# Aster32/GAN-DANet

Hardware: AMD Instinct MI355X
Metric: train samples/sec (G+D step) on 256x256 tiles (higher is better)
Workload: dtype bf16; 1 GPU; full G+D train step, 8ch 256x256 -> 1024x1024 tiles, batch 32/GPU (global 32), perceptual=on, SSIM evaluated, AdamW x2; survey_config=3, per_gpu_batch=32, global_batch=32, tile=256, parallelism=dp1

## Files before the change

### gan-danet_amd/csrc/conv3x3.hip

```cpp
#include "common.h"
#include "tile_mma.h"
#include "../../include/gandanet.h"

namespace {

using gd::acc_row;
using gd::bf16x8_native_t;
typedef unsigned int u32x4_t __attribute__((ext_vector_type(4)));

constexpr int TW = 32;
constexpr int PW = TW + 2;
constexpr int CK = 32;
constexpr int LD = CK + 8;

__global__ void pack_w_kernel(const float* __restrict__ a, long a_sm, long a_sc, long a_st, int M, int Ck, int flip,
                              int BM, int nchunks, unsigned short* __restrict__ wp, long total) {
    for (long i = (long)blockIdx.x * blockDim.x + threadIdx.x; i < total; i += (long)gridDim.x * blockDim.x) {
        const int cc = (int)(i % CK);
        long t = i / CK;
        const int mm = (int)(t % BM);
        t /= BM;
        const int tap = (int)(t % 9);
        t /= 9;
        const int chunk = (int)(t % nchunks);
        const int mt = (int)(t / nchunks);
        const int m = mt * BM + mm, c = chunk * CK + cc;
        float v = 0.f;
        if (m < M && c < Ck) v = a[(long)m * a_sm + (long)c * a_sc + (long)(flip ? 8 - tap : tap) * a_st];
        wp[i] = gd_f2bf(v);
    }
}

template <int BM, int TH, int S>
__global__ __launch_bounds__(256, 2) void conv3x3_halo_kernel(const gd_conv_desc d, const unsigned short* __restrict__ wp,
                                                             int tiles_x, int nchunks) {
    constexpr int WAVES_M = 2, WAVES_N = 2;
    constexpr int TM = BM / (32 * WAVES_M);
    constexpr int TN = TH / WAVES_N;
    constexpr int PH = S * (TH - 1) + 3;
    constexpr int PWk = S * (TW - 1) + 3;
    constexpr int NPIX = PH * PWk;
    constexpr int WCHUNKS = 3 * BM * CK / 8;
    constexpr int WPT = WCHUNKS / 256;
    static_assert(WCHUNKS % 256 == 0, "weight stage must divide evenly");

    __shared__ __attribute__((aligned(16))) unsigned short patch[NPIX * LD];
    __shared__ __attribute__((aligned(16))) unsigned short wts[3 * BM * LD];

    const int tid = threadIdx.x, lane = tid & 63, wave = tid >> 6;
    const int r = lane & 31, h = lane >> 5;
    const int wm = wave >> 1, wn = wave & 1;
    const int b = blockIdx.z;
    const int mt = blockIdx.y;
    const int ty = blockIdx.x / tiles_x, tx = blockIdx.x - ty * tiles_x;
    const int y0 = ty * TH, x0 = tx * TW;
    const int H = d.Hi, W = d.Wi;
    const int Ho = d.Ho, Wo = d.Wo;
    const long HW = (long)H * W, HWo = (long)Ho * Wo;
    const float* ximg = d.x + (long)b * d.x_bs;

    f32x16_t acc[TM][TN];
#pragma unroll
    for (int i = 0; i < TM; ++i)
#pragma unroll
        for (int j = 0; j < TN; ++j)
#pragma unroll
            for (int e = 0; e < 16; ++e) acc[i][j][e] = 0.f;

    const unsigned short* wbase = wp + (long)mt * nchunks * 9 * BM * CK;
    u32x4_t wreg[WPT];
    auto load_w = [&](int chunk, int ky) {
        const u32x4_t* src = reinterpret_cast<const u32x4_t*>(wbase + ((long)chunk * 9 + ky * 3) * BM * CK);
#pragma unroll
        for (int i = 0; i < WPT; ++i) wreg[i] = src[tid + i * 256];
    };
    auto store_w = [&]() {
#pragma unroll
        for (int i = 0; i < WPT; ++i) {
            const int v = tid + i * 256;
            const int row = v >> 2, q = v & 3;
            *reinterpret_cast<u32x4_t*>(wts + row * LD + q * 8) = wreg[i];
        }
    };

    for (int chunk = 0; chunk < nchunks; ++chunk) {
        const int c0 = chunk * CK;
        load_w(chunk, 0);
        for (int w = tid; w < 2 * NPIX; w += 256) {
            const int half = w >= NPIX ? 1 : 0;
            const int pix = w - half * NPIX;
            const int py = pix / PWk, px = pix - py * PWk;
            const int iy = S * y0 - 1 + py, ix = S * x0 - 1 + px;
            const bool inside = iy >= 0 && iy < H && ix >= 0 && ix < W;
            const int cb = c0 + half * 16;
            const float* p = ximg + (long)cb * HW + (long)iy * W + ix;
            unsigned int* dst = reinterpret_cast<unsigned int*>(patch + pix * LD + half * 16);
#pragma unroll
            for (int j = 0; j < 8; ++j) {
                const int c = cb + 2 * j;
                float v0 = 0.f, v1 = 0.f;
                if (inside) {
                    if (c < d.Ck) v0 = p[(long)(2 * j) * HW];
                    if (c + 1 < d.Ck) v1 = p[(long)(2 * j + 1) * HW];
                    if (d.in_scale) {
                        if (c < d.Ck) {
                            v0 = fmaf(v0, d.in_scale[c], d.in_shift[c]);
                            if (d.in_relu) v0 = fmaxf(v0, 0.f);
                        }
                        if (c + 1 < d.Ck) {
                            v1 = fmaf(v1, d.in_scale[c + 1], d.in_shift[c + 1]);
                            if (d.in_relu) v1 = fmaxf(v1, 0.f);
                        }
                    }
                }
                dst[j] = gd_pack_bf2(v0, v1);
            }
        }
        for (int ky = 0; ky < 3; ++ky) {
            store_w();
            __syncthreads();
            if (ky < 2) load_w(chunk, ky + 1);
#pragma unroll
            for (int kx = 0; kx < 3; ++kx) {
#pragma unroll
                for (int ks = 0; ks < CK / 16; ++ks) {
                    bf16x8_t fa[TM], fb[TN];
#pragma unroll
                    for (int i = 0; i < TM; ++i)
                        fa[i] = *reinterpret_cast<const bf16x8_t*>(wts + (kx * BM + wm * TM * 32 + i * 32 + r) * LD +
                                                                  ks * 16 + 8 * h);
#pragma unroll
                    for (int j = 0; j < TN; ++j)
                        fb[j] = *reinterpret_cast<const bf16x8_t*>(patch + (((wn * TN + j) * S + ky) * PWk + r * S + kx) * LD +
                                                                  ks * 16 + 8 * h);
#pragma unroll
                    for (int i = 0; i < TM; ++i)
#pragma unroll
                        for (int j = 0; j < TN; ++j)
                            acc[i][j] = __builtin_amdgcn_mfma_f32_32x32x16_bf16(
                                __builtin_bit_cast(bf16x8_native_t, fa[i]), __builtin_bit_cast(bf16x8_native_t, fb[j]),
                                acc[i][j], 0, 0, 0);
                }
            }
            __syncthreads();
        }
    }

    const float alpha = d.alpha ? *d.alpha : 1.f;
    const int ox = x0 + r;
    if (ox < Wo) {
#pragma unroll
        for (int j = 0; j < TN; ++j) {
            const int oy = y0 + wn * TN + j;
            if (oy >= Ho) continue;
            const long pn = (long)oy * Wo + ox;
#pragma unroll
            for (int i = 0; i < TM; ++i)
#pragma unroll
                for (int e = 0; e < 16; ++e) {
                    const int m = mt * BM + wm * TM * 32 + i * 32 + acc_row(e, h);
                    if (m >= d.M) continue;
                    float v = acc[i][j][e] * alpha;
                    if (d.bias) v += d.bias[m];
                    if (d.res) v += d.res[(long)b * d.res_bs + (long)m * HWo + pn];
                    if (d.act == GD_ACT_RELU) v = fmaxf(v, 0.f);
                    else if (d.act == GD_ACT_LEAKY02) v = v >= 0.f ? v : 0.2f * v;
                    float* yp = reinterpret_cast<float*>(d.y) + (long)b * d.y_bs + (long)m * HWo + pn;
                    if (d.accumulate) v += *yp;
                    *yp = v;
                }
        }
    }
}

}

static inline int pick_bm(int M, int Ck) {
    if (Ck <= CK && M > 64) return 128;
    return (M <= 64 || (M % 128 != 0 && M % 128 <= 64)) ? 64 : 128;
}

extern "C" size_t gd_conv3x3_ws_bytes(int M, int Ck) {
    const int bm = pick_bm(M, Ck);
    const long mtiles = (M + bm - 1) / bm, nchunks = (Ck + CK - 1) / CK;
    return (size_t)(mtiles * bm * nchunks * CK * 9 * 2);
}

extern "C" int gd_conv3x3_eligible(const gd_conv_desc* d) {
    if (!(d && d->ks == 3 && d->pad == 1 && d->out_layout == 0 && !d->out_bf16 && d->precision == GD_PREC_BF16 &&
          d->a_bs == 0 && (d->Mstore == 0 || d->Mstore == d->M) && d->sub_step <= 1))
        return 0;
    if (d->stride == 1) return d->Hi == d->Ho && d->Wi == d->Wo;
    return d->stride == 2 && !d->transposed && (d->Hi - 1) / 2 + 1 == d->Ho && (d->Wi - 1) / 2 + 1 == d->Wo;
}

extern "C" int gd_conv3x3(const gd_conv_desc* dp, void* ws, size_t ws_bytes, void* stream) {
    GD_CHECK_ARG(dp && ws, "gd_conv3x3: null argument");
    GD_CHECK_ARG(gd_conv3x3_eligible(dp), "gd_conv3x3: descriptor not eligible (needs 3x3, pad 1, stride 1 or forward stride 2, bf16, fp32 NCHW out)");
    const gd_conv_desc& d = *dp;
    GD_CHECK_ARG(d.B > 0 && d.B <= 65535 && d.M > 0 && d.Ck > 0 && d.Hi > 0 && d.Wi > 0, "gd_conv3x3: bad sizes");
    GD_CHECK_ARG(d.a && d.x && d.y, "gd_conv3x3: null tensor");
    GD_CHECK_ARG((d.in_scale == nullptr) == (d.in_shift == nullptr), "gd_conv3x3: in_scale/in_shift must come together");
    GD_CHECK_ARG(ws_bytes >= gd_conv3x3_ws_bytes(d.M, d.Ck), "gd_conv3x3: workspace too small");
    hipStream_t s = (hipStream_t)stream;
    const int bm = pick_bm(d.M, d.Ck);
    const int mtiles = (d.M + bm - 1) / bm, nchunks = (d.Ck + CK - 1) / CK;
    const long total = (long)mtiles * nchunks * 9 * bm * CK;
    {
        int blocks = (int)((total + 255) / 256);
        if (blocks > 2048) blocks = 2048;
        hipLaunchKernelGGL(pack_w_kernel, dim3(blocks), dim3(256), 0, s, d.a, d.a_sm, d.a_sc, d.a_st, d.M, d.Ck,
                           d.transposed ? 1 : 0, bm, nchunks, (unsigned short*)ws, total);
    }
    const int th = d.stride == 1 ? 8 : 4;
    const int tiles_x = (d.Wo + TW - 1) / TW, tiles_y = (d.Ho + th - 1) / th;
    GD_CHECK_ARG((long)tiles_x * tiles_y < (1L << 31), "gd_conv3x3: image too large");
    dim3 grid(tiles_x * tiles_y, mtiles, d.B);
    const unsigned short* wpk = (const unsigned short*)ws;
    if (d.stride == 1) {
        if (bm == 64) hipLaunchKernelGGL((conv3x3_halo_kernel<64, 8, 1>), grid, dim3(256), 0, s, d, wpk, tiles_x, nchunks);
        else hipLaunchKernelGGL((conv3x3_halo_kernel<128, 8, 1>), grid, dim3(256), 0, s, d, wpk, tiles_x, nchunks);
    } else {
        if (bm == 64) hipLaunchKernelGGL((conv3x3_halo_kernel<64, 4, 2>), grid, dim3(256), 0, s, d, wpk, tiles_x, nchunks);
        else hipLaunchKernelGGL((conv3x3_halo_kernel<128, 4, 2>), grid, dim3(256), 0, s, d, wpk, tiles_x, nchunks);
    }
    GD_LAUNCH_CHECK();
    return 0;
}

namespace {

struct NhwcConvArgs {
    const unsigned short* x;
    const unsigned short* wp;
    const float* bias;
    const unsigned short* mask;
    const unsigned short* res;
    unsigned short* y;
    float* y32;
    long y32_bs;
    int H, W, Ho, Wo, K, M, act, tiles_x, nchunks;
    float slope;
    int osplit;
    int epi_lds;
};

template <int BM, int S, int EPI = 0>
__global__ __launch_bounds__(256, 2) void conv3x3_nhwc_kernel(const NhwcConvArgs a) {
    constexpr int TH = S == 1 ? 8 : 4;
    constexpr int WAVES_M = 2, WAVES_N = 2;
    constexpr int TM = BM / (32 * WAVES_M);
    constexpr int TN = TH / WAVES_N;
    constexpr int PH = S * (TH - 1) + 3, PWk = S * (TW - 1) + 3, NPIX = PH * PWk;
    constexpr int WCHUNKS = 3 * BM * CK / 8;
    constexpr int WPT = WCHUNKS / 256;
    constexpr int NIT = (4 * NPIX + 255) / 256;
    static_assert(WCHUNKS % 256 == 0, "weight stage must divide evenly");

    __shared__ __attribute__((aligned(16))) unsigned short patch[NPIX * LD];
    __shared__ __attribute__((aligned(16))) unsigned short wts[3 * BM * LD];

    const int tid = threadIdx.x, lane = tid & 63, wave = tid >> 6;
    const int r = lane & 31, h = lane >> 5;
    const int wm = wave >> 1, wn = wave & 1;
    const int b = blockIdx.z, mt = blockIdx.y;
    const int ty = blockIdx.x / a.tiles_x, tx = blockIdx.x - ty * a.tiles_x;
    const int y0 = ty * TH, x0 = tx * TW;
    const int H = a.H, W = a.W, K = a.K;
    const unsigned short* ximg = a.x + (long)b * H * W * K;

    f32x16_t acc[TM][TN];
#pragma unroll
    for (int i = 0; i < TM; ++i)
#pragma unroll
        for (int j = 0; j < TN; ++j)
#pragma unroll
            for (int e = 0; e < 16; ++e) acc[i][j][e] = 0.f;

    const unsigned short* wbase = a.wp + (long)mt * a.nchunks * 9 * BM * CK;
    u32x4_t wreg[WPT];
    auto load_w = [&](int chunk, int ky) {
        const u32x4_t* src = reinterpret_cast<const u32x4_t*>(wbase + ((long)chunk * 9 + ky * 3) * BM * CK);
#pragma unroll
        for (int i = 0; i < WPT; ++i) wreg[i] = src[tid + i * 256];
    };
    auto store_w = [&]() {
#pragma unroll
        for (int i = 0; i < WPT; ++i) {
            const int v = tid + i * 256;
            const int row = v >> 2, q = v & 3;
            *reinterpret_cast<u32x4_t*>(wts + row * LD + q * 8) = wreg[i];
        }
    };

    unsigned int goff[NIT], inmask = 0, slotmask = 0;
    int loff[NIT];
#pragma unroll
    for (int it = 0; it < NIT; ++it) {
        const int w = tid + it * 256;
        const int pix = w >> 2, q = w & 3;
        const int py = pix / PWk, px = pix - py * PWk;
        const int iy = S * y0 - 1 + py, ix = S * x0 - 1 + px;
        const bool slot = w < 4 * NPIX;
        const bool inside = slot && iy >= 0 && iy < H && ix >= 0 && ix < W;
        loff[it] = pix * LD + q * 8;
        goff[it] = inside ? (unsigned int)(((long)iy * W + ix) * K + q * 8) : 0u;
        inmask |= inside ? (1u << it) : 0u;
        slotmask |= slot ? (1u << it) : 0u;
    }
    u32x4_t raw[NIT];
    auto load_patch = [&](int chunk) {
        const unsigned short* base = ximg + chunk * CK;
#pragma unroll
        for (int it = 0; it < NIT; ++it) {
            const int q = (tid + it * 256) & 3;
            const u32x4_t z = {0u, 0u, 0u, 0u};
            raw[it] = (((inmask >> it) & 1u) && chunk * CK + q * 8 < K) ? *reinterpret_cast<const u32x4_t*>(base + goff[it]) : z;
        }
    };
    auto store_patch = [&]() {
#pragma unroll
        for (int it = 0; it < NIT; ++it)
            if ((slotmask >> it) & 1u) *reinterpret_cast<u32x4_t*>(patch + loff[it]) = raw[it];
    };

    load_patch(0);
    store_patch();
    for (int chunk = 0; chunk < a.nchunks; ++chunk) {
        load_w(chunk, 0);
#pragma unroll
        for (int ky = 0; ky < 3; ++ky) {
            store_w();
            __syncthreads();
            if (ky == 0 && chunk + 1 < a.nchunks) load_patch(chunk + 1);
            if (ky < 2) load_w(chunk, ky + 1);
#pragma unroll
            for (int kx = 0; kx < 3; ++kx) {
#pragma unroll
                for (int ks = 0; ks < CK / 16; ++ks) {
                    bf16x8_t fa[TM], fb[TN];
#pragma unroll
                    for (int i = 0; i < TM; ++i)
                        fa[i] = *reinterpret_cast<const bf16x8_t*>(wts + (kx * BM + wm * TM * 32 + i * 32 + r) * LD +
                                                                  ks * 16 + 8 * h);
#pragma unroll
                    for (int j = 0; j < TN; ++j)
                        fb[j] = *reinterpret_cast<const bf16x8_t*>(patch + (((wn * TN + j) * S + ky) * PWk + r * S + kx) * LD +
                                                                  ks * 16 + 8 * h);
#pragma unroll
                    for (int i = 0; i < TM; ++i)
#pragma unroll
                        for (int j = 0; j < TN; ++j)
                            acc[i][j] = __builtin_amdgcn_mfma_f32_32x32x16_bf16(
                                __builtin_bit_cast(bf16x8_native_t, fa[i]), __builtin_bit_cast(bf16x8_native_t, fb[j]),
                                acc[i][j], 0, 0, 0);
                }
            }
            __syncthreads();
        }
        if (chunk + 1 < a.nchunks) store_patch();
    }

    if constexpr (EPI == 1) {
        constexpr int SLD = LD;
        static_assert(4 * 2 * 32 * SLD <= NPIX * LD, "per-wave scratch must fit in the patch image");
        unsigned short* scr = patch + wave * (2 * 32 * SLD);
        const int RS = a.osplit ? 3 * a.M : a.M;
        const int ox = x0 + r;
#pragma unroll
        for (int j = 0; j < TN; ++j) {
            const int oy = y0 + wn * TN + j;
            if (oy >= a.Ho) continue;
            const long prow = ((long)b * a.Ho + oy) * a.Wo;
#pragma unroll
            for (int i = 0; i < TM; ++i) {
                const int mbase = mt * BM + wm * TM * 32 + i * 32;
                if (mbase >= a.M) continue;
#pragma unroll
                for (int g = 0; g < 4; ++g) {
                    const int m = mbase + 8 * g + 4 * h;
                    const bool ok = ox < a.Wo && m < a.M;
                    float v[4];
#pragma unroll
                    for (int k = 0; k < 4; ++k) {
                        v[k] = acc[i][j][4 * g + k];
                        if (a.bias && ok) v[k] += a.bias[m + k];
                        if (a.act == 1) v[k] = fmaxf(v[k], 0.f);
                        else if (a.act == 2) v[k] = v[k] > 0.f ? v[k] : v[k] * a.slope;
                    }
                    if (ok) {
                        const long pbase = (prow + ox) * RS;
                        if (a.mask) {
                            const uint2 mk = *reinterpret_cast<const uint2*>(a.mask + pbase + m);
                            if (!((mk.x & 0x7FFFu) && !(mk.x & 0x8000u))) v[0] = 0.f;
                            if (!((mk.x >> 16) & 0x7FFFu) || (mk.x >> 31)) v[1] = 0.f;
                            if (!((mk.y & 0x7FFFu) && !(mk.y & 0x8000u))) v[2] = 0.f;
                            if (!((mk.y >> 16) & 0x7FFFu) || (mk.y >> 31)) v[3] = 0.f;
                        }
                        if (a.res) {
#pragma unroll
                            for (int part = 0; part < 2; ++part) {
                                if (part && !a.osplit) break;
                                const uint2 rr = *reinterpret_cast<const uint2*>(a.res + pbase + part * a.M + m);
                                v[0] += gd_bf2f((unsigned short)(rr.x & 0xFFFFu));
                                v[1] += gd_bf2f((unsigned short)(rr.x >> 16));
                                v[2] += gd_bf2f((unsigned short)(rr.y & 0xFFFFu));
                                v[3] += gd_bf2f((unsigned short)(rr.y >> 16));
                            }
                        }
                    }
                    uint2 hi, lo = make_uint2(0u, 0u);
                    if (a.osplit) {
                        gd_split_bf2(v[0], v[1], hi.x, lo.x);
                        gd_split_bf2(v[2], v[3], hi.y, lo.y);
                        *reinterpret_cast<uint2*>(scr + 32 * SLD + r * SLD + 8 * g + 4 * h) = lo;
                    } else {
                        hi.x = gd_pack_bf2(v[0], v[1]);
                        hi.y = gd_pack_bf2(v[2], v[3]);
                    }
                    *reinterpret_cast<uint2*>(scr + r * SLD + 8 * g + 4 * h) = hi;
                }
#pragma unroll
                for (int pass = 0; pass < 2; ++pass) {
                    const int px = pass * 16 + (lane >> 2), c8 = (lane & 3) * 8;
                    const int oxp = x0 + px, m = mbase + c8;
                    if (oxp < a.Wo && m < a.M) {
                        unsigned short* dst = a.y + (prow + oxp) * RS + m;
                        const u32x4_t vh = *reinterpret_cast<const u32x4_t*>(scr + px * SLD + c8);
                        *reinterpret_cast<u32x4_t*>(dst) = vh;
                        if (a.osplit) {
                            *reinterpret_cast<u32x4_t*>(dst + a.M) = *reinterpret_cast<const u32x4_t*>(scr + 32 * SLD + px * SLD + c8);
                            *reinterpret_cast<u32x4_t*>(dst + 2 * a.M) = vh;
                        }
                    }
                }
            }
        }
        return;
    }

    const int ox = x0 + r;
    if (ox < a.Wo) {
#pragma unroll
        for (int j = 0; j < TN; ++j) {
            const int oy = y0 + wn * TN + j;
            if (oy >= a.Ho) continue;
            const long pbase = (((long)b * a.Ho + oy) * a.Wo + ox) * (a.osplit ? 3 * a.M : a.M);
#pragma unroll
            for (int i = 0; i < TM; ++i)
#pragma unroll
                for (int g = 0; g < 4; ++g) {
                    const int m = mt * BM + wm * TM * 32 + i * 32 + 8 * g + 4 * h;
                    if (m >= a.M) continue;
                    float v[4];
#pragma unroll
                    for (int k = 0; k < 4; ++k) {
                        v[k] = acc[i][j][4 * g + k];
                        if (a.bias) v[k] += a.bias[m + k];
                        if (a.act == 1) v[k] = fmaxf(v[k], 0.f);
                        else if (a.act == 2) v[k] = v[k] > 0.f ? v[k] : v[k] * a.slope;
                    }
                    if (a.mask) {
                        const uint2 mk = *reinterpret_cast<const uint2*>(a.mask + pbase + m);
                        if (!((mk.x & 0x7FFFu) && !(mk.x & 0x8000u))) v[0] = 0.f;
                        if (!((mk.x >> 16) & 0x7FFFu) || (mk.x >> 31)) v[1] = 0.f;
                        if (!((mk.y & 0x7FFFu) && !(mk.y & 0x8000u))) v[2] = 0.f;
                        if (!((mk.y >> 16) & 0x7FFFu) || (mk.y >> 31)) v[3] = 0.f;
                    }
                    if (a.res) {
#pragma unroll
                        for (int part = 0; part < 2; ++part) {
                            if (part && !a.osplit) break;
                            const uint2 rr = *reinterpret_cast<const uint2*>(a.res + pbase + part * a.M + m);
                            v[0] += gd_bf2f((unsigned short)(rr.x & 0xFFFFu));
                            v[1] += gd_bf2f((unsigned short)(rr.x >> 16));
                            v[2] += gd_bf2f((unsigned short)(rr.y & 0xFFFFu));
                            v[3] += gd_bf2f((unsigned short)(rr.y >> 16));
                        }
                    }
                    if (a.y32) {
                        float* yp = a.y32 + (long)b * a.y32_bs + (long)m * a.Ho * a.Wo + (long)oy * a.Wo + ox;
#pragma unroll
                        for (int k = 0; k < 4; ++k) yp[(long)k * a.Ho * a.Wo] = v[k];
                        continue;
                    }
                    uint2 o;
                    if (a.osplit) {
                        uint2 lo;
                        gd_split_bf2(v[0], v[1], o.x, lo.x);
                        gd_split_bf2(v[2], v[3], o.y, lo.y);
                        *reinterpret_cast<uint2*>(a.y + pbase + a.M + m) = lo;
                        *reinterpret_cast<uint2*>(a.y + pbase + 2 * a.M + m) = o;
                    } else {
                        o.x = gd_pack_bf2(v[0], v[1]);
                        o.y = gd_pack_bf2(v[2], v[3]);
                    }
                    *reinterpret_cast<uint2*>(a.y + pbase + m) = o;
                }
        }
    }
}

struct NhwcDgrad2Args {
    const unsigned short* dy;
    const unsigned short* wp;
    const unsigned short* act;
    unsigned short* dx;
    int H, W, Ho, Wo, K, M, tiles_x, nchunks;
    float slope;
    int split;
};

__global__ __launch_bounds__(256, 2) void conv3x3_nhwc_dgrad2_kernel(const NhwcDgrad2Args a) {
    constexpr int BM = 64, TH = 4;
    constexpr int TN = TH / 2;
    constexpr int PH = TH + 1, PWd = TW + 1, NPIX = PH * PWd;
    constexpr int WPT = 3 * BM * CK / 8 / 256;
    constexpr int NIT = (4 * NPIX + 255) / 256;

    __shared__ __attribute__((aligned(16))) unsigned short patch[NPIX * LD];
    __shared__ __attribute__((aligned(16))) unsigned short wts[3 * BM * LD];

    const int tid = threadIdx.x, lane = tid & 63, wave = tid >> 6;
    const int r = lane & 31, h = lane >> 5;
    const int wm = wave >> 1, wn = wave & 1;
    const int b = blockIdx.z, mt = blockIdx.y;
    const int ty = blockIdx.x / a.tiles_x, tx = blockIdx.x - ty * a.tiles_x;
    const int u0 = ty * TH, v0 = tx * TW;
    const int Ho = a.Ho, Wo = a.Wo, M = a.M;
    const unsigned short* dyimg = a.dy + (long)b * Ho * Wo * M;

    f32x16_t acc[4][TN];
#pragma unroll
    for (int c = 0; c < 4; ++c)
#pragma unroll
        for (int j = 0; j < TN; ++j)
#pragma unroll
            for (int e = 0; e < 16; ++e) acc[c][j][e] = 0.f;

    const unsigned short* wbase = a.wp + (long)mt * a.nchunks * 9 * BM * CK;
    u32x4_t wreg[WPT];
    auto load_w = [&](int chunk, int ky) {
        const u32x4_t* src = reinterpret_cast<const u32x4_t*>(wbase + ((long)chunk * 9 + ky * 3) * BM * CK);
#pragma unroll
        for (int i = 0; i < WPT; ++i) wreg[i] = src[tid + i * 256];
    };
    auto store_w = [&]() {
#pragma unroll
        for (int i = 0; i < WPT; ++i) {
            const int v = tid + i * 256;
            *reinterpret_cast<u32x4_t*>(wts + (v >> 2) * LD + (v & 3) * 8) = wreg[i];
        }
    };

    unsigned int goff[NIT], inmask = 0, slotmask = 0;
    int loff[NIT];
#pragma unroll
    for (int it = 0; it < NIT; ++it) {
        const int w = tid + it * 256;
        const int pix = w >> 2, q = w & 3;
        const int py = pix / PWd, px = pix - py * PWd;
        const int iy = u0 + py, ix = v0 + px;
        const bool slot = w < 4 * NPIX;
        const bool inside = slot && iy < Ho && ix < Wo;
        loff[it] = pix * LD + q * 8;
        goff[it] = inside ? (unsigned int)(((long)iy * Wo + ix) * M + q * 8) : 0u;
        inmask |= inside ? (1u << it) : 0u;
        slotmask |= slot ? (1u << it) : 0u;
    }
    u32x4_t raw[NIT];
    auto load_patch = [&](int chunk) {
        const unsigned short* base = dyimg + chunk * CK;
#pragma unroll
        for (int it = 0; it < NIT; ++it) {
            const int q = (tid + it * 256) & 3;
            const u32x4_t z = {0u, 0u, 0u, 0u};
            raw[it] = (((inmask >> it) & 1u) && chunk * CK + q * 8 < M) ? *reinterpret_cast<const u32x4_t*>(base + goff[it]) : z;
        }
    };
    auto store_patch = [&]() {
#pragma unroll
        for (int it = 0; it < NIT; ++it)
            if ((slotmask >> it) & 1u) *reinterpret_cast<u32x4_t*>(patch + loff[it]) = raw[it];
    };

    load_patch(0);
    store_patch();
    for (int chunk = 0; chunk < a.nchunks; ++chunk) {
        load_w(chunk, 0);
#pragma unroll
        for (int ky = 0; ky < 3; ++ky) {
            store_w();
            __syncthreads();
            if (ky == 0 && chunk + 1 < a.nchunks) load_patch(chunk + 1);
            if (ky < 2) load_w(chunk, ky + 1);
            const int py = (ky + 1) & 1, oy = ky == 0 ? 1 : 0;
#pragma unroll
            for (int kx = 0; kx < 3; ++kx) {
                const int px = (kx + 1) & 1, ox = kx == 0 ? 1 : 0;
#pragma unroll
                for (int ks = 0; ks < CK / 16; ++ks) {
                    const bf16x8_t fa = *reinterpret_cast<const bf16x8_t*>(wts + (kx * BM + wm * 32 + r) * LD + ks * 16 + 8 * h);
#pragma unroll
                    for (int j = 0; j < TN; ++j) {
                        const bf16x8_t fb = *reinterpret_cast<const bf16x8_t*>(
                            patch + ((wn * TN + j + oy) * PWd + r + ox) * LD + ks * 16 + 8 * h);
                        acc[2 * py + px][j] = __builtin_amdgcn_mfma_f32_32x32x16_bf16(
                            __builtin_bit_cast(bf16x8_native_t, fa), __builtin_bit_cast(bf16x8_native_t, fb),
                            acc[2 * py + px][j], 0, 0, 0);
                    }
                }
            }
            __syncthreads();
        }
        if (chunk + 1 < a.nchunks) store_patch();
    }

#pragma unroll
    for (int c = 0; c < 4; ++c) {
        const int py = c >> 1, px = c & 1;
        const int X = 2 * (v0 + r) + px;
        if (X >= a.W) continue;
#pragma unroll
        for (int j = 0; j < TN; ++j) {
            const int Y = 2 * (u0 + wn * TN + j) + py;
            if (Y >= a.H) continue;
            const long pbase = (((long)b * a.H + Y) * a.W + X) * (a.split ? 3 * a.K : a.K);
#pragma unroll
            for (int g = 0; g < 4; ++g) {
                const int m = mt * BM + wm * 32 + 8 * g + 4 * h;
                if (m >= a.K) continue;
                float v[4];
#pragma unroll
                for (int k = 0; k < 4; ++k) v[k] = acc[c][j][4 * g + k];
                if (a.act) {
                    const uint2 mk = *reinterpret_cast<const uint2*>(a.act + pbase + m);
                    if (!((mk.x & 0x7FFFu) && !(mk.x & 0x8000u))) v[0] *= a.slope;
                    if (!((mk.x >> 16) & 0x7FFFu) || (mk.x >> 31)) v[1] *= a.slope;
                    if (!((mk.y & 0x7FFFu) && !(mk.y & 0x8000u))) v[2] *= a.slope;
                    if (!((mk.y >> 16) & 0x7FFFu) || (mk.y >> 31)) v[3] *= a.slope;
                }
                uint2 o;
                if (a.split) {
                    uint2 lo;
                    gd_split_bf2(v[0], v[1], o.x, lo.x);
                    gd_split_bf2(v[2], v[3], o.y, lo.y);
                    *reinterpret_cast<uint2*>(a.dx + pbase + a.K + m) = lo;
                    *reinterpret_cast<uint2*>(a.dx + pbase + 2 * a.K + m) = o;
                } else {
                    o.x = gd_pack_bf2(v[0], v[1]);
                    o.y = gd_pack_bf2(v[2], v[3]);
                }
                *reinterpret_cast<uint2*>(a.dx + pbase + m) = o;
            }
        }
    }
}

}

extern "C" int gd_conv3x3_nhwc_pack(const float* w, int Cout, int Cin, int transposed, void* ws, size_t ws_bytes,
                                    void* stream) {
    GD_CHECK_ARG(w && ws && Cout > 0 && Cin > 0 && transposed >= 0 && transposed <= 2, "gd_conv3x3_nhwc_pack: bad arguments");
    const int M = transposed ? Cin : Cout, K = transposed ? Cout : Cin;
    GD_CHECK_ARG(ws_bytes >= gd_conv3x3_ws_bytes(M, K), "gd_conv3x3_nhwc_pack: workspace too small");
    const int bm = transposed == 2 ? 64 : pick_bm(M, K);
    const int mtiles = (M + bm - 1) / bm, nchunks = (K + CK - 1) / CK;
    const long total = (long)mtiles * nchunks * 9 * bm * CK;
    int blocks = (int)((total + 255) / 256);
    if (blocks > 2048) blocks = 2048;
    const long sm = transposed ? 9 : (long)Cin * 9, sc = transposed ? (long)Cin * 9 : 9;
    hipLaunchKernelGGL(pack_w_kernel, dim3(blocks), dim3(256), 0, (hipStream_t)stream, w, sm, sc, 1L, M, K,
                       transposed == 1 ? 1 : 0, bm, nchunks, (unsigned short*)ws, total);
    GD_LAUNCH_CHECK();
    return 0;
}

static int nhwc_conv_launch(const void* x, const void* wpack, const float* bias, const void* mask, const void* res,
                            void* y, int B, int H, int W, int K, int M, int stride, int act, float slope, void* stream,
                            float* y32 = nullptr, long y32_bs = 0, int osplit = 0) {
    NhwcConvArgs a;
    static const int epi_env = getenv("GD_NHWC_EPI_LDS") ? atoi(getenv("GD_NHWC_EPI_LDS")) : 1;
    a.y32 = y32; a.y32_bs = y32_bs; a.osplit = osplit; a.epi_lds = epi_env;
    a.x = (const unsigned short*)x; a.wp = (const unsigned short*)wpack; a.bias = bias;
    a.mask = (const unsigned short*)mask; a.res = (const unsigned short*)res; a.y = (unsigned short*)y;
    a.H = H; a.W = W; a.K = K; a.M = M; a.act = act; a.slope = slope;
    a.Ho = (H - 1) / stride + 1; a.Wo = (W - 1) / stride + 1;
    const int bm = pick_bm(M, K);
    const int mtiles = (M + bm - 1) / bm;
    a.nchunks = (K + CK - 1) / CK;
    a.tiles_x = (a.Wo + TW - 1) / TW;
    const int th = stride == 1 ? 8 : 4;
    const int tiles_y = (a.Ho + th - 1) / th;
    dim3 grid(a.tiles_x * tiles_y, mtiles, B);
    hipStream_t s = (hipStream_t)stream;
    if (!a.y32 && a.epi_lds) {
        if (stride == 1) {
            if (bm == 64) hipLaunchKernelGGL((conv3x3_nhwc_kernel<64, 1, 1>), grid, dim3(256), 0, s, a);
            else hipLaunchKernelGGL((conv3x3_nhwc_kernel<128, 1, 1>), grid, dim3(256), 0, s, a);
        } else {
            if (bm == 64) hipLaunchKernelGGL((conv3x3_nhwc_kernel<64, 2, 1>), grid, dim3(256), 0, s, a);
            else hipLaunchKernelGGL((conv3x3_nhwc_kernel<128, 2, 1>), grid, dim3(256), 0, s, a);
        }
    } else if (stride == 1) {
        if (bm == 64) hipLaunchKernelGGL((conv3x3_nhwc_kernel<64, 1>), grid, dim3(256), 0, s, a);
        else hipLaunchKernelGGL((conv3x3_nhwc_kernel<128, 1>), grid, dim3(256), 0, s, a);
    } else {
        if (bm == 64) hipLaunchKernelGGL((conv3x3_nhwc_kernel<64, 2>), grid, dim3(256), 0, s, a);
        else hipLaunchKernelGGL((conv3x3_nhwc_kernel<128, 2>), grid, dim3(256), 0, s, a);
    }
    GD_LAUNCH_CHECK();
    return 0;
}

extern "C" int gd_conv3x3_nhwc(const void* x, const void* wpack, const float* bias, const void* mask, const void* res,
                               void* y, int B, int H, int W, int K, int M, int relu, int split, void* stream) {
    GD_CHECK_ARG(x && wpack && y, "gd_conv3x3_nhwc: null pointer");
    GD_CHECK_ARG(B > 0 && B <= 65535 && H > 0 && W > 0 && K > 0 && M > 0 && K % 8 == 0 && M % 8 == 0,
                 "gd_conv3x3_nhwc: channel counts must be multiples of 8");
    GD_CHECK_ARG((long)H * W * K < (1L << 31) && (long)H * W * M * (split ? 3 : 1) < (1L << 31), "gd_conv3x3_nhwc: image too large");
    return nhwc_conv_launch(x, wpack, bias, mask, res, y, B, H, W, K, M, 1, relu ? 1 : 0, 0.f, stream, nullptr, 0, split ? 1 : 0);
}

extern "C" int gd_conv3x3_nhwc_f32out(const void* x, const void* wpack, const float* bias, float* y32, long y_bs, int B, int H,
                                      int W, int K, int M, int relu, void* stream) {
    GD_CHECK_ARG(x && wpack && y32, "gd_conv3x3_nhwc_f32out: null pointer");
    GD_CHECK_ARG(B > 0 && B <= 65535 && H > 0 && W > 0 && K > 0 && M > 0 && K % 8 == 0 && M % 4 == 0 && y_bs >= (long)M * H * W,
                 "gd_conv3x3_nhwc_f32out: K must be a multiple of 8, M of 4");
    GD_CHECK_ARG((long)H * W * K < (1L << 31), "gd_conv3x3_nhwc_f32out: image too large");
    return nhwc_conv_launch(x, wpack, bias, nullptr, nullptr, nullptr, B, H, W, K, M, 1, relu ? 1 : 0, 0.f, stream, y32, y_bs);
}

extern "C" int gd_conv3x3_nhwc_s2(const void* x, const void* wpack, const float* bias, void* y, int B, int H, int W, int K,
                                  int M, int act, float slope, int split, void* stream) {
    GD_CHECK_ARG(x && wpack && y, "gd_conv3x3_nhwc_s2: null pointer");
    GD_CHECK_ARG(B > 0 && B <= 65535 && H > 0 && W > 0 && K > 0 && M > 0 && K % 8 == 0 && M % 8 == 0 && act >= 0 && act <= 2,
                 "gd_conv3x3_nhwc_s2: channel counts must be multiples of 8, act in 0..2");
    GD_CHECK_ARG((long)H * W * K < (1L << 31) && (long)H * W * M * (split ? 3 : 1) < (1L << 31), "gd_conv3x3_nhwc_s2: image too large");
    return nhwc_conv_launch(x, wpack, bias, nullptr, nullptr, y, B, H, W, K, M, 2, act, slope, stream, nullptr, 0, split ? 1 : 0);
}

extern "C" int gd_conv3x3_nhwc_s2_dgrad(const void* dy, const void* wpack_t, const void* act_out, float slope, void* dx,
                                        int B, int H, int W, int K, int M, int split, void* stream) {
    GD_CHECK_ARG(dy && wpack_t && dx, "gd_conv3x3_nhwc_s2_dgrad: null pointer");
    GD_CHECK_ARG(B > 0 && B <= 65535 && H > 0 && W > 0 && K > 0 && M > 0 && K % 8 == 0 && M % 8 == 0,
                 "gd_conv3x3_nhwc_s2_dgrad: channel counts must be multiples of 8");
    GD_CHECK_ARG((long)H * W * K * (split ? 3 : 1) < (1L << 31) && (long)H * W * M < (1L << 31), "gd_conv3x3_nhwc_s2_dgrad: image too large");
    NhwcDgrad2Args a;
    a.split = split ? 1 : 0;
    a.dy = (const unsigned short*)dy; a.wp = (const unsigned short*)wpack_t; a.act = (const unsigned short*)act_out;
    a.dx = (unsigned short*)dx; a.H = H; a.W = W; a.K = K; a.M = M; a.slope = slope;
    a.Ho = (H - 1) / 2 + 1; a.Wo = (W - 1) / 2 + 1;
    a.nchunks = (M + CK - 1) / CK;
    a.tiles_x = (a.Wo + TW - 1) / TW;
    const int tiles_y = (a.Ho + 3) / 4;
    dim3 grid(a.tiles_x * tiles_y, (K + 63) / 64, B);
    hipLaunchKernelGGL(conv3x3_nhwc_dgrad2_kernel, grid, dim3(256), 0, (hipStream_t)stream, a);
    GD_LAUNCH_CHECK();
    return 0;
}

namespace {

typedef short s16x4_t __attribute__((ext_vector_type(4)));
constexpr int WTH = 4;
constexpr int WPH = WTH + 2;
constexpr int WNPIX = WPH * PW;
constexpr int DYLD = WTH * TW + 8;

struct WgradArgs {
    const unsigned short* dy16;
    const float* dy; long dy_bs;
    const float* x; long x_bs;
    const unsigned short* x16; int x16_ld;
    const float* in_scale; const float* in_shift; int in_relu;
    float* dw;
    float* part;
    int B, M, Ck, H, W, Ho, Wo;
    int tiles_x, tiles_y, tiles_per_split;
};
typedef float f32x4u_t __attribute__((ext_vector_type(4), aligned(4)));

__device__ __forceinline__ s16x4_t lds_tr_read(const unsigned short* p) {
    return __builtin_amdgcn_ds_read_tr16_b64_v4i16((__attribute__((address_space(3))) s16x4_t*)p);
}

#ifndef GD_WGRAD_PIPED_MINW
#define GD_WGRAD_PIPED_MINW 1
#endif
template <int NW, int S, bool CS, bool PIPED = false, bool ORD = false>
__global__ __launch_bounds__(NW * 64, PIPED ? GD_WGRAD_PIPED_MINW : 2) void conv3x3_wgrad_kernel(const WgradArgs a) {
    constexpr int BM = CS ? 32 : 32 * NW, NT = 64 * NW, NCH = CS ? NW : 1;
    constexpr int PHk = S * (WTH - 1) + 3, PWk = S * (TW - 1) + 3, NPIXk = PHk * PWk;
    __shared__ __attribute__((aligned(16))) unsigned short dys[BM * DYLD];
    __shared__ __attribute__((aligned(16))) unsigned short patch[NCH * NPIXk * LD];

    const int tid = threadIdx.x, lane = tid & 63, wave = tid >> 6;
    const int r = lane & 31, h = lane >> 5;
    const int c0 = blockIdx.x * CK * NCH;
    const int m0 = blockIdx.y * BM;
    const long HW = (long)a.H * a.W;
    const long HWo = (long)a.Ho * a.Wo;
    const int ntiles = a.B * a.tiles_y * a.tiles_x;
    const int t_begin = blockIdx.z * a.tiles_per_split;
    const int t_end = min(ntiles, t_begin + a.tiles_per_split);

    f32x16_t acc[9];
#pragma unroll
    for (int t = 0; t < 9; ++t)
#pragma unroll
        for (int e = 0; e < 16; ++e) acc[t][e] = 0.f;

    const int li = lane & 15, tq = li >> 2, tp = li & 3, tg = (lane >> 4) & 1;
    const bool vec_ok = (a.Wo % 4) == 0;

    constexpr bool piped = PIPED;
    constexpr int NDY = PIPED ? (BM * 32 + NT - 1) / NT : 1;
    constexpr int NXI = PIPED ? (4 * NCH * NPIXk + NT - 1) / NT : 1;
    uint2 rdy[NDY];
    u32x4_t rxp[NXI];
    auto load_regs = [&](int t) {
        const int b = t / (a.tiles_y * a.tiles_x);
        const int rem = t - b * (a.tiles_y * a.tiles_x);
        const int ty_ = rem / a.tiles_x, tx_ = rem - ty_ * a.tiles_x;
        const int y0 = ty_ * WTH, x0 = tx_ * TW;
#pragma unroll
        for (int k = 0; k < NDY; ++k) {
            const int idx = tid + k * NT;
            const int m = idx >> 5, v = idx & 31;
            const int yy = y0 + (v >> 3), xx = x0 + (v & 7) * 4;
            uint2 w = make_uint2(0u, 0u);
            if (idx < BM * 32 && m0 + m < a.M && yy < a.Ho) {
                const unsigned short* p = a.dy16 + ((long)b * a.M + m0 + m) * HWo + (long)yy * a.Wo + xx;
                if (vec_ok && xx + 3 < a.Wo) {
                    w = *reinterpret_cast<const uint2*>(p);
                } else {
                    unsigned int e0 = xx + 0 < a.Wo ? p[0] : 0u, e1 = xx + 1 < a.Wo ? p[1] : 0u;
                    unsigned int e2 = xx + 2 < a.Wo ? p[2] : 0u, e3 = xx + 3 < a.Wo ? p[3] : 0u;
                    w.x = e0 | (e1 << 16);
                    w.y = e2 | (e3 << 16);
                }
            }
            rdy[k] = w;
        }
#pragma unroll
        for (int k = 0; k < NXI; ++k) {
            const int w = tid + k * NT;
            const int oc = w / NPIXk;
            const int q = oc & 3, chk = oc >> 2;
            const int pix = w - oc * NPIXk;
            const int py = pix / PWk, px = pix - py * PWk;
            const int iy = S * y0 - 1 + py, ix = S * x0 - 1 + px;
            const int cb = c0 + chk * CK + q * 8;
            u32x4_t v = {0u, 0u, 0u, 0u};
            if (w < 4 * NCH * NPIXk && iy >= 0 && iy < a.H && ix >= 0 && ix < a.W && cb < a.x16_ld)
                v = *reinterpret_cast<const u32x4_t*>(a.x16 + (((long)b * a.H + iy) * a.W + ix) * a.x16_ld + cb);
            rxp[k] = v;
        }
    };
    auto store_regs = [&]() {
#pragma unroll
        for (int k = 0; k < NDY; ++k) {
            const int idx = tid + k * NT;
            if (idx < BM * 32) *reinterpret_cast<uint2*>(dys + (idx >> 5) * DYLD + (idx & 31) * 4) = rdy[k];
        }
#pragma unroll
        for (int k = 0; k < NXI; ++k) {
            const int w = tid + k * NT;
            if (w < 4 * NCH * NPIXk) {
                const int oc = w / NPIXk;
                const int pix = w - oc * NPIXk;
                *reinterpret_cast<u32x4_t*>(patch + ((oc >> 2) * NPIXk + pix) * LD + (oc & 3) * 8) = rxp[k];
            }
        }
    };
    if constexpr (piped) {
        if (t_begin < t_end) load_regs(t_begin);
    }

    for (int t = t_begin; t < t_end; ++t) {
        const int b = t / (a.tiles_y * a.tiles_x);
        const int rem = t - b * (a.tiles_y * a.tiles_x);
        const int ty_ = rem / a.tiles_x, tx_ = rem - ty_ * a.tiles_x;
        const int y0 = ty_ * WTH, x0 = tx_ * TW;
        const float* dyb = a.dy + (long)b * a.dy_bs;
        const float* xb = a.x + (long)b * a.x_bs;

        if constexpr (piped) {
            store_regs();
        } else {
#pragma unroll 4
        for (int k = 0; k < 16 / (CS ? NW : 1) + (CS && (16 % NW) ? 1 : 0); ++k) {
            const int idx = tid + k * NT;
            if (CS && idx >= 32 * 32) break;
            const int m = idx >> 5, v = idx & 31;
            const int yy = y0 + (v >> 3), xx = x0 + (v & 7) * 4;
            if (a.dy16) {
                uint2 w = make_uint2(0u, 0u);
                if (m0 + m < a.M && yy < a.Ho) {
                    const unsigned short* p = a.dy16 + ((long)b * a.M + m0 + m) * HWo + (long)yy * a.Wo + xx;
                    if (vec_ok && xx + 3 < a.Wo) {
                        w = *reinterpret_cast<const uint2*>(p);
                    } else {
                        unsigned int e0 = xx + 0 < a.Wo ? p[0] : 0u, e1 = xx + 1 < a.Wo ? p[1] : 0u;
                        unsigned int e2 = xx + 2 < a.Wo ? p[2] : 0u, e3 = xx + 3 < a.Wo ? p[3] : 0u;
                        w.x = e0 | (e1 << 16);
                        w.y = e2 | (e3 << 16);
                    }
                }
                *reinterpret_cast<uint2*>(dys + m * DYLD + v * 4) = w;
                continue;
            }
            float4 f = make_float4(0.f, 0.f, 0.f, 0.f);
            if (m0 + m < a.M && yy < a.Ho) {
                const float* p = dyb + (long)(m0 + m) * HWo + (long)yy * a.Wo + xx;
                if (vec_ok && xx + 3 < a.Wo) {
                    f = *reinterpret_cast<const float4*>(p);
                } else {
// ... 236 lines not shown
```

Before: 38.36 samples/s.

## Stream conv weights directly from global into a register ring and double-buffer patches

Removes the LDS weight staging in the 3x3 NHWC conv and transposed-conv kernels. Each wave now loads its A-fragments straight from global memory into a register ring that is prefetched several k-steps ahead. The input patch is double-buffered in LDS for stride 1, which cuts the per-ky __syncthreads down to one barrier per chunk. Occupancy for BM=64 stride-1 is raised to 3 blocks/SM via launch bounds. The trade-offs are more register pressure and global weight traffic per wave, plus more LDS for the second patch buffer.

```diff
diff --git a/gan-danet_amd/csrc/conv3x3.hip b/gan-danet_amd/csrc/conv3x3.hip
--- a/gan-danet_amd/csrc/conv3x3.hip
+++ b/gan-danet_amd/csrc/conv3x3.hip
@@ -246,19 +246,19 @@
 };
 
 template <int BM, int S, int EPI = 0>
-__global__ __launch_bounds__(256, 2) void conv3x3_nhwc_kernel(const NhwcConvArgs a) {
+__global__ __launch_bounds__(256, (BM == 64 && S == 1) ? 3 : 2) void conv3x3_nhwc_kernel(const NhwcConvArgs a) {
     constexpr int TH = S == 1 ? 8 : 4;
     constexpr int WAVES_M = 2, WAVES_N = 2;
     constexpr int TM = BM / (32 * WAVES_M);
     constexpr int TN = TH / WAVES_N;
     constexpr int PH = S * (TH - 1) + 3, PWk = S * (TW - 1) + 3, NPIX = PH * PWk;
-    constexpr int WCHUNKS = 3 * BM * CK / 8;
-    constexpr int WPT = WCHUNKS / 256;
     constexpr int NIT = (4 * NPIX + 255) / 256;
-    static_assert(WCHUNKS % 256 == 0, "weight stage must divide evenly");
-
-    __shared__ __attribute__((aligned(16))) unsigned short patch[NPIX * LD];
-    __shared__ __attribute__((aligned(16))) unsigned short wts[3 * BM * LD];
+    constexpr int NSTEP = 9 * (CK / 16);
+    constexpr int RING = TM * TN >= 8 ? 3 : 6;
+    constexpr int NBUF = S == 1 ? 2 : 1;
+    static_assert(NSTEP % RING == 0, "the ring slot of a k-step must not depend on the chunk");
+
+    __shared__ __attribute__((aligned(16))) unsigned short patch[NBUF * NPIX * LD];
 
     const int tid = threadIdx.x, lane = tid & 63, wave = tid >> 6;
     const int r = lane & 31, h = lane >> 5;
@@ -278,19 +278,13 @@
             for (int e = 0; e < 16; ++e) acc[i][j][e] = 0.f;
 
     const unsigned short* wbase = a.wp + (long)mt * a.nchunks * 9 * BM * CK;
-    u32x4_t wreg[WPT];
-    auto load_w = [&](int chunk, int ky) {
-        const u32x4_t* src = reinterpret_cast<const u32x4_t*>(wbase + ((long)chunk * 9 + ky * 3) * BM * CK);
-#pragma unroll
-        for (int i = 0; i < WPT; ++i) wreg[i] = src[tid + i * 256];
-    };
-    auto store_w = [&]() {
-#pragma unroll
-        for (int i = 0; i < WPT; ++i) {
-            const int v = tid + i * 256;
-            const int row = v >> 2, q = v & 3;
-            *reinterpret_cast<u32x4_t*>(wts + row * LD + q * 8) = wreg[i];
-        }
+    const unsigned int wlane = (unsigned int)(((wm * TM * 32 + r) * CK + 8 * h) * 2);
+    const int glast = a.nchunks * 9 - 1;
+    bf16x8_t wq[RING][TM];
+    auto load_a = [&](int slot, int g, int ks) {
+        const char* src = reinterpret_cast<const char*>(wbase + (long)(g < glast ? g : glast) * (BM * CK));
+#pragma unroll
+        for (int i = 0; i < TM; ++i) wq[slot][i] = *reinterpret_cast<const bf16x8_t*>(src + wlane + (i * 32 * CK + ks * 16) * 2);
     };
 
     unsigned int goff[NIT], inmask = 0, slotmask = 0;
@@ -304,67 +298,69 @@
         const bool slot = w < 4 * NPIX;
         const bool inside = slot && iy >= 0 && iy < H && ix >= 0 && ix < W;
         loff[it] = pix * LD + q * 8;
-        goff[it] = inside ? (unsigned int)(((long)iy * W + ix) * K + q * 8) : 0u;
+        goff[it] = inside ? (unsigned int)((((long)iy * W + ix) * K + q * 8) * 2) : 0u;
         inmask |= inside ? (1u << it) : 0u;
         slotmask |= slot ? (1u << it) : 0u;
     }
     u32x4_t raw[NIT];
+    auto item_live = [&](int it, int chunk) { return ((inmask >> it) & 1u) && chunk * CK + ((tid + it * 256) & 3) * 8 < K; };
     auto load_patch = [&](int chunk) {
-        const unsigned short* base = ximg + chunk * CK;
-#pragma unroll
-        for (int it = 0; it < NIT; ++it) {
-            const int q = (tid + it * 256) & 3;
-            const u32x4_t z = {0u, 0u, 0u, 0u};
-            raw[it] = (((inmask >> it) & 1u) && chunk * CK + q * 8 < K) ? *reinterpret_cast<const u32x4_t*>(base + goff[it]) : z;
-        }
+        const char* base = reinterpret_cast<const char*>(ximg);
+#pragma unroll
+        for (int it = 0; it < NIT; ++it)
+            raw[it] = *reinterpret_cast<const u32x4_t*>(base + (item_live(it, chunk) ? goff[it] + (unsigned int)(chunk * CK * 2) : 0u));
     };
-    auto store_patch = [&]() {
+    auto store_patch = [&](unsigned short* img, int chunk) {
+        const u32x4_t z = {0u, 0u, 0u, 0u};
 #pragma unroll
         for (int it = 0; it < NIT; ++it)
-            if ((slotmask >> it) & 1u) *reinterpret_cast<u32x4_t*>(patch + loff[it]) = raw[it];
+            if ((slotmask >> it) & 1u) *reinterpret_cast<u32x4_t*>(img + loff[it]) = item_live(it, chunk) ? raw[it] : z;
     };
 
     load_patch(0);
-    store_patch();
+#pragma unroll
+    for (int s = 0; s < RING; ++s) load_a(s, s / (CK / 16), s % (CK / 16));
+    store_patch(patch, 0);
     for (int chunk = 0; chunk < a.nchunks; ++chunk) {
-        load_w(chunk, 0);
+        const unsigned short* img = patch + (NBUF == 2 ? (chunk & 1) * (NPIX * LD) : 0) + (wn * TN * S * PWk + r * S) * LD + 8 * h;
+        __syncthreads();
+        if (chunk + 1 < a.nchunks) load_patch(chunk + 1);
 #pragma unroll
         for (int ky = 0; ky < 3; ++ky) {
-            store_w();
-            __syncthreads();
-            if (ky == 0 && chunk + 1 < a.nchunks) load_patch(chunk + 1);
-            if (ky < 2) load_w(chunk, ky + 1);
 #pragma unroll
             for (int kx = 0; kx < 3; ++kx) {
 #pragma unroll
                 for (int ks = 0; ks < CK / 16; ++ks) {
-                    bf16x8_t fa[TM], fb[TN];
-#pragma unroll
-                    for (int i = 0; i < TM; ++i)
-                        fa[i] = *reinterpret_cast<const bf16x8_t*>(wts + (kx * BM + wm * TM * 32 + i * 32 + r) * LD +
-                                                                  ks * 16 + 8 * h);
+                    constexpr int KS = CK / 16;
+                    const int s = (ky * 3 + kx) * KS + ks;
+                    bf16x8_t fb[TN];
 #pragma unroll
                     for (int j = 0; j < TN; ++j)
-                        fb[j] = *reinterpret_cast<const bf16x8_t*>(patch + (((wn * TN + j) * S + ky) * PWk + r * S + kx) * LD +
-                                                                  ks * 16 + 8 * h);
+                        fb[j] = *reinterpret_cast<const bf16x8_t*>(img + ((j * S + ky) * PWk + kx) * LD + ks * 16);
 #pragma unroll
                     for (int i = 0; i < TM; ++i)
 #pragma unroll
                         for (int j = 0; j < TN; ++j)
                             acc[i][j] = __builtin_amdgcn_mfma_f32_32x32x16_bf16(
-                                __builtin_bit_cast(bf16x8_native_t, fa[i]), __builtin_bit_cast(bf16x8_native_t, fb[j]),
+                                __builtin_bit_cast(bf16x8_native_t, wq[s % RING][i]), __builtin_bit_cast(bf16x8_native_t, fb[j]),
                                 acc[i][j], 0, 0, 0);
-                }
-            }
+                    load_a(s % RING, chunk * 9 + (s + RING) / KS, (s + RING) % KS);
+                    __builtin_amdgcn_sched_barrier(0);
+                }
+            }
+        }
+        if constexpr (NBUF == 2) {
+            if (chunk + 1 < a.nchunks) store_patch(patch + ((chunk + 1) & 1) * (NPIX * LD), chunk + 1);
+        } else {
             __syncthreads();
-        }
-        if (chunk + 1 < a.nchunks) store_patch();
+            if (chunk + 1 < a.nchunks) store_patch(patch, chunk + 1);
+        }
     }
 
     if constexpr (EPI == 1) {
         constexpr int SLD = LD;
         static_assert(4 * 2 * 32 * SLD <= NPIX * LD, "per-wave scratch must fit in the patch image");
-        unsigned short* scr = patch + wave * (2 * 32 * SLD);
+        unsigned short* scr = patch + (NBUF == 2 ? (a.nchunks & 1) * (NPIX * LD) : 0) + wave * (2 * 32 * SLD);
         const int RS = a.osplit ? 3 * a.M : a.M;
         const int ox = x0 + r;
 #pragma unroll
@@ -420,6 +416,7 @@
                     }
                     *reinterpret_cast<uint2*>(scr + r * SLD + 8 * g + 4 * h) = hi;
                 }
+                __builtin_amdgcn_wave_barrier();
 #pragma unroll
                 for (int pass = 0; pass < 2; ++pass) {
                     const int px = pass * 16 + (lane >> 2), c8 = (lane & 3) * 8;
@@ -434,6 +431,7 @@
                         }
                     }
                 }
+                __builtin_amdgcn_wave_barrier();
             }
         }
         return;
@@ -515,11 +513,12 @@
     constexpr int BM = 64, TH = 4;
     constexpr int TN = TH / 2;
     constexpr int PH = TH + 1, PWd = TW + 1, NPIX = PH * PWd;
-    constexpr int WPT = 3 * BM * CK / 8 / 256;
     constexpr int NIT = (4 * NPIX + 255) / 256;
-
-    __shared__ __attribute__((aligned(16))) unsigned short patch[NPIX * LD];
-    __shared__ __attribute__((aligned(16))) unsigned short wts[3 * BM * LD];
+    constexpr int KS = CK / 16, NSTEP = 9 * KS;
+    constexpr int RING = 6;
+    static_assert(NSTEP % RING == 0, "the ring slot of a k-step must not depend on the chunk");
+
+    __shared__ __attribute__((aligned(16))) unsigned short patch[2 * NPIX * LD];
 
     const int tid = threadIdx.x, lane = tid & 63, wave = tid >> 6;
     const int r = lane & 31, h = lane >> 5;
@@ -539,18 +538,12 @@
             for (int e = 0; e < 16; ++e) acc[c][j][e] = 0.f;
 
     const unsigned short* wbase = a.wp + (long)mt * a.nchunks * 9 * BM * CK;
-    u32x4_t wreg[WPT];
-    auto load_w = [&](int chunk, int ky) {
-        const u32x4_t* src = reinterpret_cast<const u32x4_t*>(wbase + ((long)chunk * 9 + ky * 3) * BM * CK);
-#pragma unroll
-        for (int i = 0; i < WPT; ++i) wreg[i] = src[tid + i * 256];
-    };
-    auto store_w = [&]() {
-#pragma unroll
-        for (int i = 0; i < WPT; ++i) {
-            const int v = tid + i * 256;
-            *reinterpret_cast<u32x4_t*>(wts + (v >> 2) * LD + (v & 3) * 8) = wreg[i];
-        }
+    const unsigned int wlane = (unsigned int)(((wm * 32 + r) * CK + 8 * h) * 2);
+    const int glast = a.nchunks * 9 - 1;
+    bf16x8_t wq[RING];
+    auto load_a = [&](int slot, int g, int ks) {
+        const char* src = reinterpret_cast<const char*>(wbase + (long)(g < glast ? g : glast) * (BM * CK));
+        wq[slot] = *reinterpret_cast<const bf16x8_t*>(src + wlane + ks * 32);
     };
 
     unsigned int goff[NIT], inmask = 0, slotmask = 0;
@@ -564,56 +557,57 @@
         const bool slot = w < 4 * NPIX;
         const bool inside = slot && iy < Ho && ix < Wo;
         loff[it] = pix * LD + q * 8;
-        goff[it] = inside ? (unsigned int)(((long)iy * Wo + ix) * M + q * 8) : 0u;
+        goff[it] = inside ? (unsigned int)((((long)iy * Wo + ix) * M + q * 8) * 2) : 0u;
         inmask |= inside ? (1u << it) : 0u;
         slotmask |= slot ? (1u << it) : 0u;
     }
     u32x4_t raw[NIT];
+    auto item_live = [&](int it, int chunk) { return ((inmask >> it) & 1u) && chunk * CK + ((tid + it * 256) & 3) * 8 < M; };
     auto load_patch = [&](int chunk) {
-        const unsigned short* base = dyimg + chunk * CK;
-#pragma unroll
-        for (int it = 0; it < NIT; ++it) {
-            const int q = (tid + it * 256) & 3;
-            const u32x4_t z = {0u, 0u, 0u, 0u};
-            raw[it] = (((inmask >> it) & 1u) && chunk * CK + q * 8 < M) ? *reinterpret_cast<const u32x4_t*>(base + goff[it]) : z;
-        }
+        const char* base = reinterpret_cast<const char*>(dyimg);
+#pragma unroll
+        for (int it = 0; it < NIT; ++it)
+            raw[it] = *reinterpret_cast<const u32x4_t*>(base + (item_live(it, chunk) ? goff[it] + (unsigned int)(chunk * CK * 2) : 0u));
     };
-    auto store_patch = [&]() {
+    auto store_patch = [&](unsigned short* img, int chunk) {
+        const u32x4_t z = {0u, 0u, 0u, 0u};
 #pragma unroll
         for (int it = 0; it < NIT; ++it)
-            if ((slotmask >> it) & 1u) *reinterpret_cast<u32x4_t*>(patch + loff[it]) = raw[it];
+            if ((slotmask >> it) & 1u) *reinterpret_cast<u32x4_t*>(img + loff[it]) = item_live(it, chunk) ? raw[it] : z;
     };
 
     load_patch(0);
-    store_patch();
+#pragma unroll
+    for (int s = 0; s < RING; ++s) load_a(s, s / KS, s % KS);
+    store_patch(patch, 0);
     for (int chunk = 0; chunk < a.nchunks; ++chunk) {
-        load_w(chunk, 0);
+        const unsigned short* img = patch + (chunk & 1) * (NPIX * LD) + (wn * TN * PWd + r) * LD + 8 * h;
+        __syncthreads();
+        if (chunk + 1 < a.nchunks) load_patch(chunk + 1);
 #pragma unroll
         for (int ky = 0; ky < 3; ++ky) {
-            store_w();
-            __syncthreads();
-            if (ky == 0 && chunk + 1 < a.nchunks) load_patch(chunk + 1);
-            if (ky < 2) load_w(chunk, ky + 1);
             const int py = (ky + 1) & 1, oy = ky == 0 ? 1 : 0;
 #pragma unroll
             for (int kx = 0; kx < 3; ++kx) {
                 const int px = (kx + 1) & 1, ox = kx == 0 ? 1 : 0;
 #pragma unroll
-                for (int ks = 0; ks < CK / 16; ++ks) {
-                    const bf16x8_t fa = *reinterpret_cast<const bf16x8_t*>(wts + (kx * BM + wm * 32 + r) * LD + ks * 16 + 8 * h);
+                for (int ks = 0; ks < KS; ++ks) {
+                    const int s = (ky * 3 + kx) * KS + ks;
+                    const bf16x8_t fa = wq[s % RING];
 #pragma unroll
                     for (int j = 0; j < TN; ++j) {
                         const bf16x8_t fb = *reinterpret_cast<const bf16x8_t*>(
-                            patch + ((wn * TN + j + oy) * PWd + r + ox) * LD + ks * 16 + 8 * h);
+                            img + ((j + oy) * PWd + ox) * LD + ks * 16);
                         acc[2 * py + px][j] = __builtin_amdgcn_mfma_f32_32x32x16_bf16(
                             __builtin_bit_cast(bf16x8_native_t, fa), __builtin_bit_cast(bf16x8_native_t, fb),
                             acc[2 * py + px][j], 0, 0, 0);
                     }
-                }
-            }
-            __syncthreads();
-        }
-        if (chunk + 1 < a.nchunks) store_patch();
+                    load_a(s % RING, chunk * 9 + (s + RING) / KS, (s + RING) % KS);
+                    __builtin_amdgcn_sched_barrier(0);
+                }
+            }
+        }
+        if (chunk + 1 < a.nchunks) store_patch(patch + ((chunk + 1) & 1) * (NPIX * LD), chunk + 1);
     }
 
 #pragma unroll
```

Result: no change. 38.28 samples/s (-0.2%).
